# Pose-Group/FAMI-Pose

Hardware: AMD Instinct MI355X
Metric: train clips/sec (5-frame 384x288 HRNet-W48) (higher is better)
Workload: dtype f32

## Files before the change

### fami-pose_amd/csrc/conv.hip

```cpp
#include "common.h"
#include <type_traits>
#include <string.h>

#include "conv_epi.h"
extern "C" int fami_conv2d_fwd_bnin_ok(int N, int H, int W, int Ci, int Co);
#include "conv_pair.h"
int fami_pair_launch(const PairCapture& c, hipStream_t s);


struct ConvArgs {
  EpiBN e;
  int emode;
  const float* x;
  const float* wp;
  float* y;
  const float* bias;
  const float* addend;
  int N, Hi, Wi, Ci, Ho, Wo, Co;
  int kh, kw, sh, pad, dil;
  int KC, NTt, relu, accumulate, P;
  unsigned x_bytes, wp_bytes;
  int xcd;
  int prio;
  int par;
// ... 2387 lines not shown
        attr2 = true;                                                                                              \
      }                                                                                                            \
      hipLaunchKernelGGL((conv3x3_lds_kernel<T, nt, ksc, 1>), grid, dim3(256), lds, s, a);                         \
    } else                                                                                                         \
    hipLaunchKernelGGL((conv3x3_lds_kernel<T, nt, ksc>), grid, dim3(256), lds, s, a);                              \
    launched = true;                                                                                               \
  }
  FAMI_LDS_CASE(3, 1) FAMI_LDS_CASE(3, 2) FAMI_LDS_CASE(3, 3) FAMI_LDS_CASE(3, 4)
  FAMI_LDS_CASE(4, 1) FAMI_LDS_CASE(4, 2) FAMI_LDS_CASE(4, 3) FAMI_LDS_CASE(4, 4)
#undef FAMI_LDS_CASE
  if (!launched) return 0;
  hipError_t e = hipGetLastError();
  if (e != hipSuccess) {
    fami_set_error(name, hipGetErrorString(e));
    return FAMI_EHIP;
  }
  return 1;
}

static bool wgrad_lin_ok(int H, int W, int Ci, int Co, int kh, int kw, int stride, int pad, int dil) {
  return stride == 1 && 2 * pad == dil * (kh - 1) && 2 * pad == dil * (kw - 1) && kh * kw > 1 && kh * kw <= 9 && W >= 4 &&
         Ci % 16 == 0 && Co % 16 == 0;
}
static bool geom_ok(int kh, int kw, int stride, int pad, int dil) {
  return kh >= 1 && kw >= 1 && kh <= 7 && kw <= 7 && (stride == 1 || stride == 2) && pad >= 0 && dil >= 1;
}
static inline int out_dim(int i, int k, int stride, int pad, int dil) {
  return (i + 2 * pad - dil * (k - 1) - 1) / stride + 1;
}

extern "C" {
int fami_dcn_tune(int mode);
int fami_bn_tune_small(long elems);

int fami_conv_tune(int mt, int nt, int ks) {
  g_force_mt = mt; g_force_nt = nt; g_force_ks = ks;
  return FAMI_OK;
}
void fami_conv_stem_tune(int on);
int fami_conv_tune_lds(int on) {
  if (on == 9000 || on == 9001) {
    fami_conv_stem_tune(on - 9000);
    return FAMI_OK;
  }
  if (on < 0) fami_conv_stem_tune(-1);
  if (on == 10 || on == 11 || on == 20 || on == 21 || on == 30 || on == 31 || (on >= 40 && on <= 42) || (on >= 52 && on <= 54) || (on >= 60 && on <= 62) || on >= 100) {
    fami_conv_t4_tune(on);
    return FAMI_OK;
  }
  g_use_lds = on < 0 ? -1 : (on ? 1 : 0);
  g_lds_sim = on == 2;
  if (on < 0) fami_conv_t4_tune(-1);
  return FAMI_OK;
}
int fami_conv_tune_wgrad_lds(int on) {
  if (on >= 30000) {
    fami_wgrad_s3_tune(on - 30000);
    return FAMI_OK;
  }
  if (on >= 20000) {
    fami_wgrad16_tune(on - 20000);
    return FAMI_OK;
  }
  if (on >= 1000) {
    g_wgrad_ps = on - 1000;
    return FAMI_OK;
// ... 20 lines not shown
  if (on > 1) g_wgrad_nsub = on - 1;
  return FAMI_OK;
}
int fami_conv_tune_xcd(int mode) {
  g_xcd = mode < 0 ? -1 : (mode & 1);
  g_xcd_w = mode < 0 ? 1 : ((mode >> 1) & 1);
  return FAMI_OK;
}
int fami_conv_tune_stages(int stages) {
  if (stages == 120 || stages == 121) {
    g_prio = stages - 120;
    return FAMI_OK;
  }
  if (stages == 110 || stages == 111) {
    g_par = stages - 110;
    return FAMI_OK;
  }
  if (stages == 100 || stages == 101) {
    g_lin_conv = stages - 100;
    return FAMI_OK;
  }
  g_stages = (stages >= 2 && stages <= 4) ? stages : 0;
  return FAMI_OK;
}
int fami_tune_reset(void) {
  fami_conv_tune(0, 0, 0);
  fami_conv_tune_lds(-1);
  fami_conv_tune_wgrad_lds(-1);
  fami_conv_tune_xcd(-1);
  g_stages = 0; g_prio = 0; g_lin_conv = 1; g_par = 1;
  g_wgrad_ps = 0; g_wgrad_mt = 0;
  fami_dcn_tune(-1);
  fami_bn_tune_small(-1);
  return FAMI_OK;
}
int fami_tune_defaults(int f32_split) {
  if (f32_split >= 0) {
    fami_conv_t4_default_split(f32_split);
    fami_wgrad_s3_default(f32_split);
  }
  return fami_tune_reset();
}

long fami_packed_weight_elems(int Co, int Ci, int kh, int kw, int mode) {
  const int kd = mode == 0 ? Ci : Co, nd = mode == 0 ? Co : Ci;
  return pack16_elems(kd, nd, kh * kw) + pack32_elems(kd, nd, kh * kw) + fami_split_image_elems(kd, nd, kh * kw);
}

int fami_pack_conv_weight_f32(const float* w_oihw, float* wp, int Co, int Ci, int kh, int kw, int mode,
                              hipStream_t s) {
  FAMI_REQUIRE(w_oihw && wp && Co > 0 && Ci > 0 && (mode == 0 || mode == 1), "fami_pack_conv_weight_f32", "bad argument");
  const int kd = mode == 0 ? Ci : Co, nd = mode == 0 ? Co : Ci;
  const long total = pack16_elems(kd, nd, kh * kw) + pack32_elems(kd, nd, kh * kw);
  hipLaunchKernelGGL(pack_w_kernel, dim3(fami_ew_grid(total)), dim3(256), 0, s, w_oihw, wp, Co, Ci, kh * kw, mode);
  FAMI_CHECK_LAUNCH("fami_pack_conv_weight_f32");
  if (fami_split_image_elems(kd, nd, kh * kw) > 0) {
    fami_pack_split_single(w_oihw, wp + total, Co, Ci, kh * kw, mode, s);
    FAMI_CHECK_LAUNCH("fami_pack_conv_weight_f32/split");
  }
  return FAMI_OK;
}

static int conv_fwd_f32_impl(const char* nm, const float* x, const float* wp, const float* bias, const float* addend,
                             float* y, int N, int H, int W, int Ci, int Co, int kh, int kw, int stride, int pad, int dil,
                             int relu, int accumulate, const EpiBN& e, hipStream_t s, const XBN& xbn = xbn_none());
int fami_conv2d_fwd_f32(const float* x, const float* wp, const float* bias, const float* addend, float* y, int N,
// ... 35 lines not shown
                             int relu, int accumulate, const EpiBN& e, hipStream_t s, const XBN& xbn) {
  FAMI_REQUIRE(x && wp && y && N > 0 && H > 0 && W > 0 && Ci > 0 && Co > 0, nm, "bad argument");
  if (!geom_ok(kh, kw, stride, pad, dil)) {
    fami_set_error(nm, "unsupported geometry");
    return FAMI_ESHAPE;
  }
  ConvArgs a;
  a.e = e; a.emode = e.slots ? e.mode : 0;
  a.x = x; a.wp = wp; a.y = y; a.bias = bias; a.addend = addend;
  a.N = N; a.Hi = H; a.Wi = W; a.Ci = Ci;
  a.Ho = out_dim(H, kh, stride, pad, dil); a.Wo = out_dim(W, kw, stride, pad, dil); a.Co = Co;
  a.kh = kh; a.kw = kw; a.sh = stride == 2 ? 1 : 0; a.pad = pad; a.dil = dil;
  a.KC = fami_cdiv(Ci, 16); a.NTt = fami_cdiv(Co, 16); a.relu = relu; a.accumulate = accumulate;
  const long P = (long)N * a.Ho * a.Wo;
  const long xb = (long)N * H * W * Ci * 4, wb = (long)kh * kw * a.KC * a.NTt * 1024;
  FAMI_REQUIRE(P > 0 && P < (1L << 31) && xb < (1L << 31) && wb < (1L << 31), nm, "tensor >= 2 GiB");
  a.P = (int)P; a.x_bytes = (unsigned)xb; a.wp_bytes = (unsigned)wb;
  if (Ci == 3 && !addend && !xbn.on) {
    const int rc = fami_try_conv_stem1(2, x, wp, bias, y, N, H, W, Ci, Co, kh, kw, stride, pad, dil, a.NTt, relu, accumulate, 1, s, nm, e);
    if (rc != 0) return rc < 0 ? rc : FAMI_OK;
  }
  if (kh == 3 && kw == 3 && stride == 1 && pad == 1 && dil == 1 && !addend) {
    const int rc = try_conv3x3_lds<float>(x, wp, bias, y, N, H, W, Ci, Co, a.KC, a.NTt, +1, relu, accumulate, 1, s, nm, e, xbn);
    if (rc != 0) return rc < 0 ? rc : FAMI_OK;
  }
  if (kh == 3 && kw == 3 && stride == 1 && pad == dil && dil > 1 && !addend && !e.slots && !xbn.on && g_use_lds != 0) {
    const int rc = fami_try_conv3x3_t4_dil(2, x, wp, bias, y, N, H, W, Ci, Co, a.KC, a.NTt, +1, relu, accumulate, 1, dil, s, nm);
    if (rc != 0) return rc < 0 ? rc : FAMI_OK;
  }
  if (xbn.on) {
    fami_set_error(nm, "input BatchNorm needs the split-product 3x3 kernel (ask fami_conv2d_xbn_ok_f32 first)");
    return FAMI_ESHAPE;
  }
  return run_igemm(a, 0, s, nm);
}
extern "C" {

static int conv_dgrad_f32_impl(const char* nm, const float* dy, const float* wp, const float* addend, float* dx, int N,
                               int H, int W, int Ci, int Co, int kh, int kw, int stride, int pad, int dil, int accumulate,
                               const EpiBN& e, hipStream_t s);
int fami_conv2d_dgrad_f32(const float* dy, const float* wp, const float* addend, float* dx, int N, int H, int W,
                          int Ci, int Co, int kh, int kw, int stride, int pad, int dil, int accumulate,
                          hipStream_t s) {
  return conv_dgrad_f32_impl("fami_conv2d_dgrad_f32", dy, wp, addend, dx, N, H, W, Ci, Co, kh, kw, stride, pad, dil,
                             accumulate, epi_none(), s);
}
int fami_conv2d_dgrad_bnstats_f32(const float* dy, const float* wp, float* dx, int N, int H, int W, int Ci, int Co,
                                  int kh, int kw, int stride, int pad, int dil, int accumulate, const float* z,
                                  const float* yrelu, const float* mean, const float* invstd, const float* gamma,
                                  const float* beta, int relu, void* slots, hipStream_t s) {
  FAMI_REQUIRE(slots && z && mean && invstd && gamma && beta && (relu != 1 || yrelu) && relu >= 0 && relu <= 2,
               "fami_conv2d_dgrad_bnstats_f32", "bad argument");
  EpiBN e = epi_none();
  e.slots = reinterpret_cast<double*>(slots); e.ns = bn_slots(Ci); e.mode = 2; e.relu = relu; e.C = Ci;
  e.z = z; e.yr = yrelu; e.mean = mean; e.invstd = invstd; e.gamma = gamma; e.beta = beta;
  return conv_dgrad_f32_impl("fami_conv2d_dgrad_bnstats_f32", dy, wp, nullptr, dx, N, H, W, Ci, Co, kh, kw, stride, pad,
                             dil, accumulate, e, s);
}
}
static int conv_dgrad_f32_impl(const char* nm, const float* dy, const float* wp, const float* addend, float* dx, int N,
                               int H, int W, int Ci, int Co, int kh, int kw, int stride, int pad, int dil, int accumulate,
                               const EpiBN& e, hipStream_t s) {
  FAMI_REQUIRE(dy && wp && dx && N > 0 && H > 0 && W > 0 && Ci > 0 && Co > 0, nm, "bad argument");
  if (!geom_ok(kh, kw, stride, pad, dil)) {
    fami_set_error(nm, "unsupported geometry");
    return FAMI_ESHAPE;
  }
  ConvArgs a;
  a.e = e; a.emode = e.slots ? e.mode : 0;
  a.x = dy; a.wp = wp; a.y = dx; a.bias = nullptr; a.addend = addend;
  a.N = N; a.Hi = out_dim(H, kh, stride, pad, dil); a.Wi = out_dim(W, kw, stride, pad, dil); a.Ci = Co;
  a.Ho = H; a.Wo = W; a.Co = Ci;
  a.kh = kh; a.kw = kw; a.sh = stride == 2 ? 1 : 0; a.pad = pad; a.dil = dil;
  a.KC = fami_cdiv(Co, 16); a.NTt = fami_cdiv(Ci, 16); a.relu = 0; a.accumulate = accumulate;
  const long P = (long)N * H * W;
  const long xb = (long)N * a.Hi * a.Wi * Co * 4, wb = (long)kh * kw * a.KC * a.NTt * 1024;
  FAMI_REQUIRE(P > 0 && P < (1L << 31) && xb < (1L << 31) && wb < (1L << 31), nm, "tensor >= 2 GiB");
  a.P = (int)P; a.x_bytes = (unsigned)xb; a.wp_bytes = (unsigned)wb;
  if (kh == 3 && kw == 3 && stride == 1 && pad == 1 && dil == 1 && !addend) {
    const int rc = try_conv3x3_lds<float>(dy, wp, nullptr, dx, N, H, W, Co, Ci, a.KC, a.NTt, -1, 0, accumulate, 1, s, nm, e);
    if (rc != 0) return rc < 0 ? rc : FAMI_OK;
  }
  if (kh == 3 && kw == 3 && stride == 1 && pad == dil && dil > 1 && !addend && !e.slots && g_use_lds != 0) {
    const int rc = fami_try_conv3x3_t4_dil(2, dy, wp, nullptr, dx, N, H, W, Co, Ci, a.KC, a.NTt, -1, 0, accumulate, 1, dil, s, nm);
    if (rc != 0) return rc < 0 ? rc : FAMI_OK;
  }
  return run_igemm(a, 1, s, nm);
}
extern "C" {

struct WgradPlan { int MT, NT, ciBlocks, coBlocks, psplit, chunk, pertap, w8; long P; };
static bool wgrad_lin_ok(int H, int W, int Ci, int Co, int kh, int kw, int stride, int pad, int dil);
static WgradPlan wgrad_plan(int N, int H, int W, int Ci, int Co, int kh, int kw, int stride, int pad, int dil, int w8 = 0) {
  WgradPlan q;
  const int Ho = out_dim(H, kh, stride, pad, dil), Wo = out_dim(W, kw, stride, pad, dil);
  q.P = (long)N * Ho * Wo;
  q.MT = pick_small(fami_cdiv(Ci, 16));
  q.NT = pick_small(fami_cdiv(Co, 16));
  if (g_wgrad_mt > 0 && g_wgrad_mt <= q.MT) q.MT = g_wgrad_mt;
  q.ciBlocks = fami_cdiv(fami_cdiv(Ci, 16), q.MT);
  q.coBlocks = fami_cdiv(fami_cdiv(Co, 16), q.NT);
  q.pertap = (kh * kw > 1 && kh * kw <= 9) ? 1 : 0;
  const long by = q.pertap ? (long)q.ciBlocks * q.coBlocks : (long)kh * kw * q.ciBlocks * q.coBlocks;
  long ps = ((q.pertap ? (g_wgrad_ps ? g_wgrad_ps : 512) : 1024) + by - 1) / by;
  q.w8 = 0;
  if (w8 == 3) w8 = 256 / by >= 16 ? 2 : 1;
  if (w8 && q.pertap && kh * kw == 9 && ps >= 9) {
    q.w8 = w8;
    const long T = (g_wgrad_ps ? g_wgrad_ps : (w8 == 2 ? 256 : 512)) / by;
    ps = T * 8 / 9;
    while (ps > 1 && ps + (ps + 7) / 8 > T) --ps;
    if (ps < 1) ps = 1;
    if (w8 == 2) ps *= 2;
  }
  const long maxps = q.pertap ? (q.P + 63) / 64 : (q.P + 255) / 256;
  if (ps > maxps) ps = maxps;
  if (ps < 1) ps = 1;
// ... 62 lines not shown
  G = (P + chunk - 1) / chunk;
  q.G = (int)G;
  q.chunk = (int)chunk;
  q.xbytes = (int)((chunk + 2 * (W + 1)) * q.xrow);
  q.lds = ((size_t)q.xbytes + (size_t)chunk * q.yrow + 16) * 4;
  q.ok = P < (1L << 31) && G < 65536;
  return q;
}

int fami_conv2d_xbn_ok(int N, int H, int W, int Ci, int Co) {
  return (g_use_lds != 0 && g_wgrad_lds && fami_conv_t4_eligible16(N, H, W, Ci, Co) &&
          fami_wgrad16_slabs(N, H, W, Ci, Co, 3, 1, 1, 1) > 0) ? 1 : 0;
}
long fami_conv2d_wgrad_workspace(int N, int H, int W, int Ci, int Co, int kh, int kw, int stride, int pad, int dil) {
  if (!geom_ok(kh, kw, stride, pad, dil)) return -1;
  const WgradPlan q = wgrad_plan(N, H, W, Ci, Co, kh, kw, stride, pad, dil);
  long need = (long)q.psplit * Co * Ci * kh * kw * (long)sizeof(float);
  const WgradLdsPlan l = wgrad_lds_plan(N, H, W, Ci, Co, kh, kw, stride, pad, dil);
  if (l.ok) {
    const long nl = (long)l.G * Co * Ci * 9 * (long)sizeof(float);
    if (nl > need) need = nl;
  }
  const WgradLdsPlan f = wgrad_lds_plan_f32(N, H, W, Ci, Co, kh, kw, stride, pad, dil);
  if (f.ok) {
    const long nl = (long)f.G * Co * Ci * 9 * (long)sizeof(float);
    if (nl > need) need = nl;
  }
  if (kh == kw) {
    const long nl = fami_wgrad16_slabs(N, H, W, Ci, Co, kh, stride, pad, dil) * Co * Ci * kh * kw * (long)sizeof(float);
    if (nl > need) need = nl;
  }
  if (kh == 3 && kw == 3 && stride == 1 && pad == 1 && dil == 1) {
    const long nl = fami_wgrad_s3_slabs(N, H, W, Ci, Co) * Co * Ci * 9 * (long)sizeof(float);
    if (nl > need) need = nl;
  }
  return need;
}

}

template <typename T>
static int wgrad_impl(const T* x, const T* dy, float* dw, float* workspace, long ws_bytes, int N, int H, int W, int Ci,
                      int Co, int kh, int kw, int stride, int pad, int dil, int accumulate, hipStream_t s,
                      const char* nm) {
  FAMI_REQUIRE(x && dy && dw && workspace && N > 0 && H > 0 && W > 0 && Ci > 0 && Co > 0, nm, "bad argument");
  if (!geom_ok(kh, kw, stride, pad, dil)) {
    fami_set_error(nm, "unsupported geometry");
    return FAMI_ESHAPE;
  }
  const bool lin = std::is_same<T, float>::value && g_wgrad_lin && wgrad_lin_ok(H, W, Ci, Co, kh, kw, stride, pad, dil);
  const WgradPlan q = wgrad_plan(N, H, W, Ci, Co, kh, kw, stride, pad, dil, !lin ? 0 : (g_wgrad_lin == 1 ? 3 : (g_wgrad_lin == 3 ? 1 : (g_wgrad_lin == 4 ? 2 : 0))));
  const long need = (long)q.psplit * Co * Ci * kh * kw * (long)sizeof(float);
  FAMI_REQUIRE(ws_bytes >= need, nm, "workspace too small");
  FAMI_REQUIRE(q.P < (1L << 31), nm, "size out of range");
  WgradArgs<T> a;
  a.x = x; a.dy = dy; a.part = workspace;
  a.N = N; a.H = H; a.W = W; a.Ci = Ci;
  a.Ho = out_dim(H, kh, stride, pad, dil); a.Wo = out_dim(W, kw, stride, pad, dil); a.Co = Co;
  a.kh = kh; a.kw = kw; a.sh = stride == 2 ? 1 : 0; a.pad = pad; a.dil = dil;
  a.P = (int)q.P; a.chunk = q.chunk; a.ciBlocks = q.ciBlocks; a.coBlocks = q.coBlocks; a.xcd = g_xcd_w; a.prio = g_prio;
  const long xb = (long)N * H * W * Ci * (long)sizeof(T), yb = q.P * Co * (long)sizeof(T);
  FAMI_REQUIRE(xb < (1L << 31) && yb < (1L << 31), nm, "tensor >= 2 GiB");
  a.x_bytes = (unsigned)xb; a.dy_bytes = (unsigned)yb;
  if (q.pertap) {
    const dim3 grid(q.w8 ? q.psplit + (q.psplit + 7) / 8 : q.psplit, q.ciBlocks * q.coBlocks), block(q.w8 ? 512 * q.w8 : kh * kw * 64);
    const size_t lin_lds = q.w8 == 2 ? (size_t)8 * q.MT * q.NT * 1024 : 0;
// ... 104 lines not shown
  if (vec && g_force_mt) { MT = g_force_mt; NT = g_force_nt ? g_force_nt : NT; KS = g_force_ks ? g_force_ks : 1; }
  const int ST = g_stages ? g_stages : 2;
  int rc;
  if (mode == 0)
    rc = vec ? launch_igemm_h<H, 0, 1>(a, MT, NT, KS, ST, s) : launch_igemm_h<H, 0, 0>(a, MT, NT, KS, 2, s);
  else
    rc = vec ? launch_igemm_h<H, 1, 1>(a, MT, NT, KS, ST, s) : launch_igemm_h<H, 1, 0>(a, MT, NT, KS, 2, s);
  if (rc != 0) {
    fami_set_error(name, "no kernel instance for tile shape");
    return FAMI_ESHAPE;
  }
  FAMI_CHECK_LAUNCH(name);
  return FAMI_OK;
}

extern "C" {

static int wgrad_f32_entry(const float* x, const float* dy, float* dw, float* workspace, long ws_bytes, int N, int H,
                           int W, int Ci, int Co, int kh, int kw, int stride, int pad, int dil, int accumulate,
                           hipStream_t s, const XBN& xbn);
int fami_conv2d_wgrad_f32(const float* x, const float* dy, float* dw, float* workspace, long ws_bytes, int N, int H,
                          int W, int Ci, int Co, int kh, int kw, int stride, int pad, int dil, int accumulate,
                          hipStream_t s) {
  return wgrad_f32_entry(x, dy, dw, workspace, ws_bytes, N, H, W, Ci, Co, kh, kw, stride, pad, dil, accumulate, s, xbn_none());
}
static int wgrad_f32_entry(const float* x, const float* dy, float* dw, float* workspace, long ws_bytes, int N, int H,
                           int W, int Ci, int Co, int kh, int kw, int stride, int pad, int dil, int accumulate,
                           hipStream_t s, const XBN& xbn) {
  if (kh == 3 && kw == 3 && stride == 1 && pad == 1 && dil == 1 && x && dy && dw && workspace) {
    const int G = fami_try_wgrad_s3(x, dy, workspace, ws_bytes, N, H, W, Ci, Co, s, "fami_conv2d_wgrad_f32", xbn);
    if (G < 0) return G;
    if (G > 0) {
      launch_reduce_taps(workspace, dw, Co, Ci, 9, G, accumulate, s);
      FAMI_CHECK_LAUNCH("fami_conv2d_wgrad_f32/reduce");
      return FAMI_OK;
    }
  }
  if (xbn.on) {
    fami_set_error("fami_conv2d_wgrad_defer_xbn_f32", "input BatchNorm needs the split-product kernel (ask fami_conv2d_xbn_ok_f32 first)");
    return FAMI_ESHAPE;
  }
  WgradLdsPlan l = g_wgrad_lds_f32 ? wgrad_lds_plan_f32(N, H, W, Ci, Co, kh, kw, stride, pad, dil) : WgradLdsPlan{0};
  if (g_wgrad_lds_f32 == 2 && l.ok &&
      (l.ciBlocks * l.coBlocks < 64 || (g_wgrad_lin && wgrad_lin_ok(H, W, Ci, Co, kh, kw, stride, pad, dil))))
    l.ok = 0;
  if (l.ok && x && dy && dw && workspace && ((reinterpret_cast<uintptr_t>(x) | reinterpret_cast<uintptr_t>(dy)) & 15) == 0) {
    const long need = (long)l.G * Co * Ci * 9 * (long)sizeof(float);
    FAMI_REQUIRE(ws_bytes >= need, "fami_conv2d_wgrad_f32", "workspace too small");
    WgradLdsArgsF a;
    a.x = x; a.dy = dy; a.part = workspace;
    a.N = N; a.H = H; a.W = W; a.Ci = Ci; a.Co = Co; a.P = N * H * W;
    a.chunk = l.chunk; a.ciBlocks = l.ciBlocks; a.coBlocks = l.coBlocks; a.xcd = g_xcd_w;
    a.CiB = 16 * l.CIT; a.CoB = 16 * l.COT; a.xrow = l.xrow; a.yrow = l.yrow; a.xfloats = l.xbytes;
    const dim3 grid(l.G, l.ciBlocks * l.coBlocks);
    bool ok = false;
#define FAMI_WF_CASE(cit, cot)                                                                                        \
  if (l.CIT == cit && l.COT == cot) {                                                                                 \
    static bool attr = false;                                                                                         \
    if (!attr) {                                                                                                      \
      (void)hipFuncSetAttribute((const void*)conv_wgrad_lds_f32_kernel<cit, cot>, hipFuncAttributeMaxDynamicSharedMemorySize, 160 * 1024); \
      attr = true;                                                                                                    \
    }                                                                                                                 \
    hipLaunchKernelGGL((conv_wgrad_lds_f32_kernel<cit, cot>), grid, dim3(512), l.lds, s, a);                          \
    ok = true;                                                                                                        \
  }
    FAMI_WF_CASE(1, 1) FAMI_WF_CASE(1, 2) FAMI_WF_CASE(1, 3) FAMI_WF_CASE(1, 4) FAMI_WF_CASE(2, 1) FAMI_WF_CASE(2, 2)
// ... 444 lines not shown
```

### fami-pose_amd/csrc/conv_epi.h

```cpp
#pragma once
#include "common.h"

struct EpiBN {
  double* slots;
  int ns, mode, relu, C;
  const float* pivot_src;
  const void* z;
  const void* yr;
  const float *mean, *invstd, *gamma, *beta;
};
static inline EpiBN epi_none() {
  EpiBN e;
  e.slots = nullptr; e.ns = 1; e.mode = 0; e.relu = 0; e.C = 0; e.pivot_src = nullptr; e.z = nullptr; e.yr = nullptr;
  e.mean = e.invstd = e.gamma = e.beta = nullptr;
  return e;
}
#if defined(__HIP_DEVICE_COMPILE__)
typedef const __attribute__((address_space(4))) EpiBN* EpiPtr;
__device__ __forceinline__ EpiPtr epi_late(unsigned off) {
  const __attribute__((address_space(4))) char* k =
      (const __attribute__((address_space(4))) char*)__builtin_amdgcn_kernarg_segment_ptr() + off;
  asm volatile("" : "+s"(k) : : "memory");
  return (EpiPtr)k;
}
// ... 75 lines not shown
int fami_try_conv3x3_t4_dil(int half_kind, const void* x, const void* wp, const float* bias, void* y, int N, int H, int W, int Ci,
                            int Co, int KC, int NTt, int sgn, int relu, int accumulate, int out_f32, int dil, hipStream_t s,
                            const char* name);
void fami_conv_t4_tune(int on);
void fami_conv_t4_default_split(int on);
int fami_conv_t4_eligible16(int N, int H, int W, int Ci, int Co);
int fami_conv_t4_eligible_s3(int N, int H, int W, int Ci, int Co);

long fami_wgrad16_slabs(int N, int H, int W, int Ci, int Co, int k, int st, int pad, int dil);
int fami_try_wgrad16(int half_kind, const void* x, const void* dy, float* part, long ws_bytes, int N, int H, int W, int Ci,
                     int Co, int k, int st, int pad, int dil, hipStream_t s, const char* name, const XBN& xbn = xbn_none());
void fami_wgrad16_tune(int on);

long fami_wgrad_s3_slabs(int N, int H, int W, int Ci, int Co);
int fami_try_wgrad_s3(const float* x, const float* dy, float* part, long ws_bytes, int N, int H, int W, int Ci, int Co,
                      hipStream_t s, const char* name, const XBN& xbn = xbn_none());
void fami_wgrad_s3_tune(int on);
void fami_wgrad_s3_default(int on);

long fami_split_image_elems(int kd, int nd, int taps);
void fami_pack_split_single(const float* w_oihw, float* split, int Co, int Ci, int taps, int mode, hipStream_t s);
void fami_pack_split_batch(const float* params, float* packed, const void* desc, int n, hipStream_t s);
int fami_try_conv3x3_t5(int half_kind, const void* x, const void* wp, const float* bias, void* y, int N, int H, int W, int Ci,
                        int Co, int KC, int NTt, int sgn, int relu, int accumulate, int out_f32, hipStream_t s,
                        const char* name, const EpiBN& epi, const XBN& xbn);
void fami_conv_t5_tune(int on);
int fami_conv_t5_eligible_s3(int N, int H, int W, int Ci, int Co);

int fami_try_conv3x3_t6(int half_kind, const void* x, const void* wp, const float* bias, void* y, int N, int H, int W, int Ci,
                        int Co, int KC, int NTt, int sgn, int relu, int accumulate, int out_f32, hipStream_t s,
                        const char* name, const EpiBN& epi, const XBN& xbn);
extern "C" int fami_conv_t6_eligible(int N, int H, int W, int Ci, int Co);
void fami_conv_t6_tune(int on);
```

### fami-pose_amd/csrc/route.h

```cpp
#pragma once
#include "../../include/fami_route.h"
extern "C" fami_route_t* fami_rt(void);

#define g_dcn_gather (fami_rt()->dcn_gather)
#define g_dcn_abl (fami_rt()->dcn_abl)
#define g_dcn_win_r (fami_rt()->dcn_win_r)
#define g_dcn_ksplit (fami_rt()->dcn_ksplit)
#define g_dcn_pf (fami_rt()->dcn_pf)
#define g_dcn_bwd2 (fami_rt()->dcn_bwd2)
#define g_dcn_bwd2_cap (fami_rt()->dcn_bwd2_cap)
#define g_dcn_bwd2_stage (fami_rt()->dcn_bwd2_stage)
#define g_dcn_bwd_abl (fami_rt()->dcn_bwd_abl)
#define g_dcn_bwd_scatter (fami_rt()->dcn_bwd_scatter)
#define g_prio (fami_rt()->prio)
#define g_lin_conv (fami_rt()->lin_conv)
#define g_par (fami_rt()->par)
#define g_force_mt (fami_rt()->force_mt)
#define g_force_nt (fami_rt()->force_nt)
#define g_force_ks (fami_rt()->force_ks)
#define g_stages (fami_rt()->stages)
#define g_use32 (fami_rt()->use32)
#define g_xcd_w (fami_rt()->xcd_w)
#define g_xcd (fami_rt()->xcd)
#define g_use_lds (fami_rt()->use_lds)
// ... 28 lines not shown
#define g_t6_rows (fami_rt()->t6_rows)
#define g_t6_min_jobs (fami_rt()->t6_min_jobs)
#define g_t6_mt (fami_rt()->t6_mt)
#define g_t7_target (fami_rt()->t7_target)
#define g_use_t7 (fami_rt()->use_t7)
#define g_t7_rows (fami_rt()->t7_rows)
#define g_t7_c64 (fami_rt()->t7_c64)
#define g_bn_in (fami_rt()->bn_in)
#define g_bwd_pair (fami_rt()->bwd_pair)
#define g_pair_wg6_target (fami_rt()->pair_wg6_target)
#define g_wg6_s2 (fami_rt()->wg6_s2)
#define g_wg6_dil (fami_rt()->wg6_dil)
#define g_wg6_c42 (fami_rt()->wg6_c42)
#define g_wg6_c4 (fami_rt()->wg6_c4)
#define g_wg6 (fami_rt()->wg6)
#define g_wg6_nu (fami_rt()->wg6_nu)
#define g_wg6_target (fami_rt()->wg6_target)
#define g_wg6_target_c4 (fami_rt()->wg6_target_c4)
#define g_wg1 (fami_rt()->wg1)
#define g_wg1_target (fami_rt()->wg1_target)
#define g_wgs (fami_rt()->wgs)
#define g_wg16_abl (fami_rt()->wg16_abl)
#define g_wg16 (fami_rt()->wg16)
#define g_wg16_bt (fami_rt()->wg16_bt)
#define g_wg16_target (fami_rt()->wg16_target)
#define g_wg16_general (fami_rt()->wg16_general)
#define g_wg16_bt18 (fami_rt()->wg16_bt18)
#define g_wgs3 (fami_rt()->wgs3)
#define g_wgs3_bt (fami_rt()->wgs3_bt)
#define g_wgs3_target (fami_rt()->wgs3_target)
#define g_wgs3_default (fami_rt()->wgs3_default)
#define g_bn_small_elems (fami_rt()->bn_small_elems)
#define g_bn2_maxg (fami_rt()->bn2_maxg)

static inline void fami_route_set_defaults(fami_route_t* q) {
  q->size = (int)sizeof(fami_route_t);
  q->dcn_gather = -1;
  q->dcn_abl = 0;
  q->dcn_win_r = 0;
  q->dcn_ksplit = 1;
  q->dcn_pf = 0;
  q->dcn_bwd2 = 1;
  q->dcn_bwd2_cap = 36;
  q->dcn_bwd2_stage = 1;
  q->dcn_bwd_abl = 0;
  q->dcn_bwd_scatter = -1;
  q->prio = 0;
  q->lin_conv = 1;
  q->par = 1;
  q->force_mt = 0;
  q->force_nt = 0;
  q->force_ks = 0;
  q->stages = 0;
  q->use32 = 1;
  q->xcd_w = 1;
  q->xcd = -1;
  q->use_lds = -1;
  q->lds_sim = 0;
  q->wgrad_nsub = 2;
  q->wgrad_ps = 0;
  q->wgrad_mt = 0;
  q->wgrad_lds = 1;
  q->wgrad_lds_f32 = 2;
  q->wgrad_lin = 1;
  q->stem1 = 1;
  q->use_t4 = 1;
// ... 19 lines not shown
  q->t6_rows = 0;
  q->t6_min_jobs = 96;
  q->t6_mt = 0;
  q->t7_target = 240;
  q->use_t7 = 1;
  q->t7_rows = 0;
  q->t7_c64 = 1;
  q->bn_in = 1;
  q->bwd_pair = 1;
  q->pair_wg6_target = 64;
  q->wg6_s2 = 1;
  q->wg6_dil = 1;
  q->wg6_c42 = 1;
  q->wg6_c4 = 1;
  q->wg6 = 1;
  q->wg6_nu = 0;
  q->wg6_target = 80;
  q->wg6_target_c4 = 160;
  q->wg1 = 1;
  q->wg1_target = 192;
  q->wgs = 1;
  q->wg16_abl = 0;
  q->wg16 = 1;
  q->wg16_bt = 0;
  q->wg16_target = 0;
  q->wg16_general = 1;
  q->wg16_bt18 = 0;
  q->wgs3 = 1;
  q->wgs3_bt = 0;
  q->wgs3_target = 0;
  q->wgs3_default = 1;
  q->bn_small_elems = 32768;
  q->bn2_maxg = 512;
}
```

### include/fami.h

```cpp
#ifndef FAMI_H
#define FAMI_H
#ifdef __cplusplus
extern "C" {
#endif

typedef void* fami_stream_t;

#include "fami_route.h"
long fami_route_size(void);
int fami_route_init(fami_route_t* route);
int fami_route_bind(fami_route_t* route);

const char* fami_version(void);
const char* fami_last_error(void);
int fami_device_info(int device, int* info, char* name, int name_len);

int fami_conv_tune(int mt, int nt, int ks);
int fami_conv_tune_lds(int on);
int fami_conv_tune_wgrad_lds(int on);
int fami_conv_tune_xcd(int mode);
int fami_conv_tune_stages(int stages);
int fami_tune_reset(void);
int fami_tune_defaults(int f32_split);
int fami_conv_t5_eligible(int N, int H, int W, int Ci, int Co);
int fami_conv_t6_eligible(int N, int H, int W, int Ci, int Co);
long fami_packed_weight_elems(int Co, int Ci, int kh, int kw, int mode);
int fami_pack_conv_weight_f32(const float* w_oihw, float* wp, int Co, int Ci, int kh, int kw, int mode,
                              fami_stream_t stream);
int fami_pack_conv_weights_batch_f32(const float* params, float* packed, const void* desc, int n, fami_stream_t stream);
int fami_conv2d_fwd_f32(const float* x, const float* wp, const float* bias, const float* addend, float* y, int N,
                        int H, int W, int Ci, int Co, int kh, int kw, int stride, int pad, int dil, int relu,
                        int accumulate, fami_stream_t stream);
int fami_conv2d_dgrad_f32(const float* dy, const float* wp, const float* addend, float* dx, int N, int H, int W,
                          int Ci, int Co, int kh, int kw, int stride, int pad, int dil, int accumulate,
                          fami_stream_t stream);
int fami_conv2d_fwd_stats_f32(const float* x, const float* wp, const float* bias, float* y, int N, int H, int W, int Ci,
                              int Co, int kh, int kw, int stride, int pad, int dil, void* slots, const float* pivot_src,
                              fami_stream_t stream);
int fami_conv2d_dgrad_bnstats_f32(const float* dy, const float* wp, float* dx, int N, int H, int W, int Ci, int Co,
                                  int kh, int kw, int stride, int pad, int dil, int accumulate, const float* z,
                                  const float* yrelu, const float* mean, const float* invstd, const float* gamma,
                                  const float* beta, int relu, void* slots, fami_stream_t stream);
long fami_conv2d_wgrad_workspace(int N, int H, int W, int Ci, int Co, int kh, int kw, int stride, int pad, int dil);
int fami_wgrad_reduce_desc_longs(void);
int fami_wgrad_reduce_batch(const long* descs, int n, fami_stream_t stream);
int fami_conv2d_wgrad_defer_f32(const float* x, const float* dy, float* dw, float* workspace, long ws_bytes, int N,
                                int H, int W, int Ci, int Co, int kh, int kw, int stride, int pad, int dil,
                                int accumulate, long* desc_out, fami_stream_t stream);
int fami_conv2d_wgrad_f32(const float* x, const float* dy, float* dw, float* workspace, long ws_bytes, int N, int H,
                          int W, int Ci, int Co, int kh, int kw, int stride, int pad, int dil, int accumulate,
                          fami_stream_t stream);

long fami_bn_workspace(int C);
int fami_bn_stats_f32(const float* x, long P, int C, float* mean, float* invstd, float* running_mean,
                      float* running_var, float momentum, float eps, float* ws, fami_stream_t stream);
int fami_bn_train_fwd_f32(const float* x, const float* residual, float* y, const float* gamma, const float* beta,
                          float* mean, float* invstd, float* running_mean, float* running_var, long P, int C,
                          int relu, float momentum, float eps, float* ws, fami_stream_t stream);
// ... 446 lines not shown
```

### include/fami_route.h

```cpp
#ifndef FAMI_ROUTE_H
#define FAMI_ROUTE_H
#ifdef __cplusplus
extern "C" {
#endif

typedef struct fami_route_t {
  int size;
  int  dcn_gather;
  int  dcn_abl;
  int  dcn_win_r;
  int  dcn_ksplit;
  int  dcn_pf;
  int  dcn_bwd2;
  int  dcn_bwd2_cap;
  int  dcn_bwd2_stage;
  int  dcn_bwd_abl;
  int  dcn_bwd_scatter;
  int  prio;
  int  lin_conv;
  int  par;
  int  force_mt;
  int  force_nt;
  int  force_ks;
  int  stages;
// ... 32 lines not shown
  int  t6_rows;
  int  t6_min_jobs;
  int  t6_mt;
  int  t7_target;
  int  use_t7;
  int  t7_rows;
  int  t7_c64;
  int  bn_in;
  int  bwd_pair;
  int  pair_wg6_target;
  int  wg6_s2;
  int  wg6_dil;
  int  wg6_c42;
  int  wg6_c4;
  int  wg6;
  int  wg6_nu;
  int  wg6_target;
  int  wg6_target_c4;
  int  wg1;
  int  wg1_target;
  int  wgs;
  int  wg16_abl;
  int  wg16;
  int  wg16_bt;
  int  wg16_target;
  int  wg16_general;
  int  wg16_bt18;
  int  wgs3;
  int  wgs3_bt;
  int  wgs3_target;
  int  wgs3_default;
  long bn_small_elems;
  int  bn2_maxg;
} fami_route_t;

#ifdef __cplusplus
}
#endif
#endif
```

Baseline: 90.95.

## Add dedicated pointwise 1x1 conv kernels for forward, dgrad and weight gradient

Adds a specialized MFMA-based 1x1 convolution kernel with swizzled LDS staging and a fused bias/addend/relu/BN-stats epilogue, used for forward and data-gradient. It also adds a 1x1 weight-gradient kernel that writes per-block partial slabs, which are then reduced. By default only the weight-gradient path for large 64x64-channel layers is eligible; forward and dgrad need the tune mode raised. The aim is to replace the generic implicit-GEMM path for these layers at the cost of extra workspace and a reduction pass.

Measured after the change: 90.93. No clear change (-0.0%).

```diff
diff --git a/fami-pose_amd/csrc/conv.hip b/fami-pose_amd/csrc/conv.hip
--- a/fami-pose_amd/csrc/conv.hip
+++ b/fami-pose_amd/csrc/conv.hip
@@ -2443,6 +2443,7 @@
 extern "C" {
 int fami_dcn_tune(int mode);
 int fami_bn_tune_small(long elems);
+int fami_conv_pw_tune(int mode);
 
 int fami_conv_tune(int mt, int nt, int ks) {
   g_force_mt = mt; g_force_nt = nt; g_force_ks = ks;
@@ -2529,6 +2530,7 @@
   g_wgrad_ps = 0; g_wgrad_mt = 0;
   fami_dcn_tune(-1);
   fami_bn_tune_small(-1);
+  fami_conv_pw_tune(-1);
   return FAMI_OK;
 }
 int fami_tune_defaults(int f32_split) {
@@ -2630,6 +2632,10 @@
     fami_set_error(nm, "input BatchNorm needs the split-product 3x3 kernel (ask fami_conv2d_xbn_ok_f32 first)");
     return FAMI_ESHAPE;
   }
+  if (kh == 1 && kw == 1 && stride == 1 && pad == 0 && dil == 1 && pack32_elems(Ci, Co, 1) > 0) {
+    const int rc = fami_try_conv_pw(x, wp + pack16_elems(Ci, Co, 1), bias, addend, y, P, Ci, Co, relu, accumulate, 0, e, s, nm);
+    if (rc != 0) return rc < 0 ? rc : FAMI_OK;
+  }
   return run_igemm(a, 0, s, nm);
 }
 extern "C" {
@@ -2681,6 +2687,10 @@
   }
   if (kh == 3 && kw == 3 && stride == 1 && pad == dil && dil > 1 && !addend && !e.slots && g_use_lds != 0) {
     const int rc = fami_try_conv3x3_t4_dil(2, dy, wp, nullptr, dx, N, H, W, Co, Ci, a.KC, a.NTt, -1, 0, accumulate, 1, dil, s, nm);
+    if (rc != 0) return rc < 0 ? rc : FAMI_OK;
+  }
+  if (kh == 1 && kw == 1 && stride == 1 && pad == 0 && dil == 1 && pack32_elems(Co, Ci, 1) > 0 && !fami_pair_capture()) {
+    const int rc = fami_try_conv_pw(dy, wp + pack16_elems(Co, Ci, 1), nullptr, addend, dx, P, Co, Ci, 0, accumulate, 1, e, s, nm);
     if (rc != 0) return rc < 0 ? rc : FAMI_OK;
   }
   return run_igemm(a, 1, s, nm);
@@ -2809,6 +2819,10 @@
   }
   if (kh == 3 && kw == 3 && stride == 1 && pad == 1 && dil == 1) {
     const long nl = fami_wgrad_s3_slabs(N, H, W, Ci, Co) * Co * Ci * 9 * (long)sizeof(float);
+    if (nl > need) need = nl;
+  }
+  if (kh == 1 && kw == 1 && stride == 1 && pad == 0 && dil == 1) {
+    const long nl = fami_pw_wgrad_slabs((long)N * H * W, Ci, Co) * Co * Ci * (long)sizeof(float);
     if (nl > need) need = nl;
   }
   return need;
@@ -2979,6 +2993,15 @@
     if (G < 0) return G;
     if (G > 0) {
       launch_reduce_taps(workspace, dw, Co, Ci, 9, G, accumulate, s);
+      FAMI_CHECK_LAUNCH("fami_conv2d_wgrad_f32/reduce");
+      return FAMI_OK;
+    }
+  }
+  if (kh == 1 && kw == 1 && stride == 1 && pad == 0 && dil == 1 && x && dy && dw && workspace && !xbn.on && !fami_pair_capture()) {
+    const int G = fami_try_wgrad_pw(x, dy, workspace, ws_bytes, (long)N * H * W, Ci, Co, s, "fami_conv2d_wgrad_f32");
+    if (G < 0) return G;
+    if (G > 0) {
+      launch_reduce_plain(workspace, dw, Co, Ci, 1, G, accumulate, s);
       FAMI_CHECK_LAUNCH("fami_conv2d_wgrad_f32/reduce");
       return FAMI_OK;
     }
diff --git a/fami-pose_amd/csrc/conv_epi.h b/fami-pose_amd/csrc/conv_epi.h
--- a/fami-pose_amd/csrc/conv_epi.h
+++ b/fami-pose_amd/csrc/conv_epi.h
@@ -131,3 +131,9 @@
                         const char* name, const EpiBN& epi, const XBN& xbn);
 extern "C" int fami_conv_t6_eligible(int N, int H, int W, int Ci, int Co);
 void fami_conv_t6_tune(int on);
+
+int fami_try_conv_pw(const float* x, const float* wp32, const float* bias, const float* addend, float* y, long P, int K,
+                     int N, int relu, int accumulate, int dir, const EpiBN& epi, hipStream_t s, const char* name);
+long fami_pw_wgrad_slabs(long P, int Ci, int Co);
+int fami_try_wgrad_pw(const float* x, const float* dy, float* part, long ws_bytes, long P, int Ci, int Co, hipStream_t s,
+                      const char* name);
diff --git a/fami-pose_amd/csrc/conv_pw.hip b/fami-pose_amd/csrc/conv_pw.hip
--- /dev/null
+++ b/fami-pose_amd/csrc/conv_pw.hip
@@ -0,0 +1,373 @@
+#include "common.h"
+#include "conv_epi.h"
+
+typedef float f32x16 __attribute__((ext_vector_type(16)));
+#define PW_OOB 0x80000000u
+
+
+#define PW_MP 128
+struct PwArgs {
+  EpiBN e;
+  int emode;
+  const float* x;
+  const float* wp;
+  float* y;
+  const float* bias;
+  const float* addend;
+  int P, K, N, KC8, NT32, relu, accumulate;
+  unsigned x_bytes, wp_bytes;
+};
+
+template <int KFIX>
+__global__ __launch_bounds__(256, 2) void conv_pw_f32(PwArgs p) {
+  __shared__ __attribute__((aligned(16))) float lds[PW_MP * 64 + 64 * 64 + 512];
+  float* xs = lds;
+  float* ws = lds + PW_MP * 64;
+  float* ered = ws + 64 * 64;
+  const int t = threadIdx.x;
+  const int lane = t & 63;
+  const int wave = __builtin_amdgcn_readfirstlane(t >> 6);
+  const int col = lane & 31, h = lane >> 5;
+  const int K = KFIX ? KFIX : p.K;
+  const int nkc = (K + 63) >> 6, nnc = (p.NT32 + 1) >> 1;
+  const int m0 = blockIdx.x * PW_MP;
+  const int emode = p.emode;
+  const __amdgpu_buffer_rsrc_t rx = __builtin_amdgcn_make_buffer_rsrc((void*)p.x, 0, (int)p.x_bytes, 0x00020000);
+  const __amdgpu_buffer_rsrc_t rw = __builtin_amdgcn_make_buffer_rsrc((void*)p.wp, 0, (int)p.wp_bytes, 0x00020000);
+
+  u32x4 xr[8], wr[4];
+  const int spx = t >> 4, sc4 = t & 15;
+  const unsigned xv = (unsigned)(((m0 + spx) * K + sc4 * 4) * 4);
+  auto load_x = [&](int kc) {
+    const bool cv = kc * 64 + sc4 * 4 < K;
+#pragma unroll
+    for (int i = 0; i < 8; ++i) {
+      const unsigned o = cv ? xv + (unsigned)((i * 16 * K + kc * 64) * 4) : PW_OOB;
+      xr[i] = __builtin_amdgcn_raw_buffer_load_b128(rx, o, 0, 0);
+    }
+  };
+  auto store_x = [&]() {
+#pragma unroll
+    for (int i = 0; i < 8; ++i) {
+      const int px = i * 16 + spx;
+      *reinterpret_cast<u32x4*>(xs + px * 64 + ((sc4 ^ (px & 15)) << 2)) = xr[i];
+    }
+  };
+  auto load_w = [&](int nc, int kc) {
+#pragma unroll
+    for (int i = 0; i < 4; ++i) {
+      const int idx = i * 256 + t;
+      const int k8 = kc * 8 + (idx >> 7), ntg = nc * 2 + ((idx >> 6) & 1);
+      const unsigned o = (k8 < p.KC8 && ntg < p.NT32) ? (unsigned)(((k8 * p.NT32 + ntg) * 64 + (idx & 63)) * 16) : PW_OOB;
+      wr[i] = __builtin_amdgcn_raw_buffer_load_b128(rw, o, 0, 0);
+    }
+  };
+  auto store_w = [&]() {
+#pragma unroll
+    for (int i = 0; i < 4; ++i) *reinterpret_cast<u32x4*>(ws + (i * 256 + t) * 4) = wr[i];
+  };
+
+  f32x16 acc[2], tot[2];
+  const float* xfrag = xs + (wave * 32 + col) * 64;
+  const int xsw = col & 15;
+
+  const bool restage_x = nkc > 1;
+  load_x(0);
+  load_w(0, 0);
+  const int nsteps = nnc * nkc;
+  int nc = 0, kc = 0;
+#pragma unroll 1
+  for (int step = 0; step < nsteps; ++step) {
+    __syncthreads();
+    if (restage_x || step == 0) store_x();
+    store_w();
+    __syncthreads();
+    int nc1 = nc, kc1 = kc + 1;
+    if (kc1 == nkc) { kc1 = 0; ++nc1; }
+    if (step + 1 < nsteps) {
+      if (restage_x) load_x(kc1);
+      load_w(nc1, kc1);
+    }
+#pragma unroll
+    for (int r = 0; r < 16; ++r) acc[0][r] = acc[1][r] = 0.f;
+#pragma unroll
+    for (int ks = 0; ks < 8; ++ks) {
+      const f32x4 a = *reinterpret_cast<const f32x4*>(xfrag + (((ks * 2 + h) ^ xsw) << 2));
+      const f32x4 b0 = *reinterpret_cast<const f32x4*>(ws + ((ks * 2 + 0) * 64 + lane) * 4);
+      const f32x4 b1 = *reinterpret_cast<const f32x4*>(ws + ((ks * 2 + 1) * 64 + lane) * 4);
+#pragma unroll
+      for (int u = 0; u < 4; ++u) {
+        acc[0] = __builtin_amdgcn_mfma_f32_32x32x2f32(b0[u], a[u], acc[0], 0, 0, 0);
+        acc[1] = __builtin_amdgcn_mfma_f32_32x32x2f32(b1[u], a[u], acc[1], 0, 0, 0);
+      }
+    }
+    if (restage_x) {
+      if (kc == 0) {
+        tot[0] = acc[0];
+        tot[1] = acc[1];
+      } else {
+        tot[0] += acc[0];
+        tot[1] += acc[1];
+      }
+      if (kc == nkc - 1) {
+        acc[0] = tot[0];
+        acc[1] = tot[1];
+      }
+    }
+    if (kc == nkc - 1) {
+#pragma unroll
+      for (int nt = 0; nt < 2; ++nt) {
+        if (nc * 2 + nt >= p.NT32) break;
+        __syncthreads();
+        {
+          const int lp = wave * 32 + col;
+#pragma unroll
+          for (int q = 0; q < 4; ++q) {
+            const f32x4 v = {acc[nt][4 * q], acc[nt][4 * q + 1], acc[nt][4 * q + 2], acc[nt][4 * q + 3]};
+            *reinterpret_cast<f32x4*>(ws + lp * 32 + (((2 * q + h) ^ (lp & 7)) << 2)) = v;
+          }
+        }
+        __syncthreads();
+        const int u = t & 7;
+        const int co = (nc * 2 + nt) * 32 + u * 4;
+        f32x4 bv = {0.f, 0.f, 0.f, 0.f}, ek = {0.f, 0.f, 0.f, 0.f}, es = {0.f, 0.f, 0.f, 0.f}, eq = {0.f, 0.f, 0.f, 0.f};
+        if (p.bias) {
+#pragma unroll
+          for (int r = 0; r < 4; ++r) bv[r] = p.bias[co + r];
+        }
+        if (emode) {
+          EpiPtr e = epi_late(__builtin_offsetof(PwArgs, e));
+          const float* ps = e->pivot_src;
+          if (ps) {
+#pragma unroll
+            for (int r = 0; r < 4; ++r) ek[r] = ps[co + r];
+          }
+        }
+#pragma unroll
+        for (int pass = 0; pass < 4; ++pass) {
+          const int lp = pass * 32 + (t >> 3);
+          const int m = m0 + lp;
+          if (m >= p.P) continue;
+          f32x4 v = *reinterpret_cast<const f32x4*>(ws + lp * 32 + ((u ^ (lp & 7)) << 2));
+          const long idx = (long)m * p.N + co;
+          v += bv;
+          if (p.addend) v += *reinterpret_cast<const f32x4*>(p.addend + idx);
+          if (p.relu) {
+#pragma unroll
+            for (int r = 0; r < 4; ++r) v[r] = fmaxf(v[r], 0.f);
+          }
+          if (p.accumulate) v += *reinterpret_cast<const f32x4*>(p.y + idx);
+          if (emode) {
+            const f32x4 d = v - ek;
+            es += d;
+#pragma unroll
+            for (int r = 0; r < 4; ++r) eq[r] = __builtin_fmaf(d[r], d[r], eq[r]);
+          }
+          *reinterpret_cast<f32x4*>(p.y + idx) = v;
+        }
+        if (emode) {
+#pragma unroll
+          for (int r = 0; r < 4; ++r) {
+#pragma unroll
+            for (int o = 8; o < 64; o <<= 1) {
+              es[r] += __shfl_xor(es[r], o, 64);
+              eq[r] += __shfl_xor(eq[r], o, 64);
+            }
+          }
+          if (lane < 8) {
+            *reinterpret_cast<f32x4*>(ered + wave * 128 + nt * 32 + u * 4) = es;
+            *reinterpret_cast<f32x4*>(ered + wave * 128 + 64 + nt * 32 + u * 4) = eq;
+          }
+        }
+      }
+      if (emode) {
+        __syncthreads();
+        if (t < 128) {
+          EpiPtr e = epi_late(__builtin_offsetof(PwArgs, e));
+          const int st = t >> 6, c = t & 63;
+          const int co = nc * 64 + c;
+          if (co < p.N) {
+            const int eC = e->C;
+            double* srow = e->slots + (long)((int)blockIdx.x % e->ns) * 2 * eC;
+            const float v = (ered[t] + ered[128 + t]) + (ered[256 + t] + ered[384 + t]);
+            unsafeAtomicAdd(srow + st * eC + co, (double)v);
+            if (st == 0 && blockIdx.x == 0) bn_slots_pivot(e->slots, eC)[co] = e->pivot_src ? e->pivot_src[co] : 0.f;
+          }
+        }
+      }
+    }
+    nc = nc1;
+    kc = kc1;
+  }
+}
+
+static bool pw_shape_ok(long P, int Ci, int Co, int dir) {
+  if (P <= 0 || Ci <= 0 || Co <= 0) return false;
+  if (dir == 2) {
+    return Ci % 32 == 0 && Co % 32 == 0 && (Ci / 32) * (Co / 32) <= 16 && Ci + Co <= 512 && (P + 128) * (Ci > Co ? Ci : Co) * 4 < (1L << 31);
+  }
+  const int K = dir == 0 ? Ci : Co, N = dir == 0 ? Co : Ci;
+  return K % 16 == 0 && N % 32 == 0 && N >= 64 && (P + PW_MP) * (K > N ? K : N) * 4 < (1L << 31);
+}
+static bool pw_eligible(long P, int Ci, int Co, int dir) {
+  if (g_pw_f32 == 0 || !pw_shape_ok(P, Ci, Co, dir)) return false;
+  if (g_pw_f32 >= 2) return true;
+  return dir == 2 && P >= 65536 && Ci == 64 && Co == 64;
+}
+
+extern "C" {
+int fami_conv_pw_tune(int mode) {
+  g_pw_f32 = mode < 0 ? 1 : (mode > 2 ? 2 : mode);
+  return FAMI_OK;
+}
+int fami_conv_pw_eligible_f32(int N, int H, int W, int Ci, int Co, int direction) {
+  if (direction < 0 || direction > 2 || N <= 0 || H <= 0 || W <= 0) return 0;
+  return pw_eligible((long)N * H * W, Ci, Co, direction) ? 1 : 0;
+}
+}
+
+int fami_try_conv_pw(const float* x, const float* wp32, const float* bias, const float* addend, float* y, long P, int K,
+                     int N, int relu, int accumulate, int dir, const EpiBN& epi, hipStream_t s, const char* name) {
+  if (!pw_eligible(P, dir == 0 ? K : N, dir == 0 ? N : K, dir)) return 0;
+  if (epi.slots && epi.mode != 1) return 0;
+  const uintptr_t al = reinterpret_cast<uintptr_t>(x) | reinterpret_cast<uintptr_t>(y) | reinterpret_cast<uintptr_t>(wp32) |
+                       reinterpret_cast<uintptr_t>(addend);
+  if (al & 15) return 0;
+  PwArgs a;
+  a.e = epi; a.emode = epi.slots ? 1 : 0;
+  a.x = x; a.wp = wp32; a.y = y; a.bias = bias; a.addend = addend;
+  a.P = (int)P; a.K = K; a.N = N; a.KC8 = K / 8; a.NT32 = N / 32; a.relu = relu; a.accumulate = accumulate;
+  a.x_bytes = (unsigned)(P * K * 4); a.wp_bytes = (unsigned)((long)a.KC8 * a.NT32 * 1024);
+  const dim3 grid(fami_cdiv(P, PW_MP));
+  if (K == 64) hipLaunchKernelGGL(conv_pw_f32<64>, grid, dim3(256), 0, s, a);
+  else if (K == 256) hipLaunchKernelGGL(conv_pw_f32<256>, grid, dim3(256), 0, s, a);
+  else hipLaunchKernelGGL(conv_pw_f32<0>, grid, dim3(256), 0, s, a);
+  FAMI_CHECK_LAUNCH(name);
+  return 1;
+}
+
+struct PwWgArgs {
+  const float* x;
+  const float* dy;
+  float* part;
+  int P, Ci, Co, run, cpx;
+  unsigned x_bytes, dy_bytes;
+};
+#define PW_WG_NLD 16
+
+template <int TPW>
+__global__ __launch_bounds__(256) void conv_pw_wgrad_f32(PwWgArgs p) {
+  extern __shared__ __attribute__((aligned(16))) float wlds[];
+  const int t = threadIdx.x;
+  const int lane = t & 63;
+  const int wave = __builtin_amdgcn_readfirstlane(t >> 6);
+  const int col = lane & 31, h = lane >> 5;
+  const int Ci = p.Ci, Co = p.Co, cpx = p.cpx;
+  const int q0 = blockIdx.x * p.run;
+  const int qend = min(q0 + p.run, p.P);
+  float* xt = wlds;
+  float* yt = wlds + cpx * Ci;
+  const __amdgpu_buffer_rsrc_t rx = __builtin_amdgcn_make_buffer_rsrc((void*)p.x, 0, (int)p.x_bytes, 0x00020000);
+  const __amdgpu_buffer_rsrc_t ry = __builtin_amdgcn_make_buffer_rsrc((void*)p.dy, 0, (int)p.dy_bytes, 0x00020000);
+  const int nx = (cpx * Ci) >> 10, nld = nx + ((cpx * Co) >> 10);
+  const unsigned tv = (unsigned)t * 16u;
+
+  u32x4 sr[PW_WG_NLD];
+  auto load = [&](int q) {
+    const unsigned xq = (unsigned)(q * Ci * 4), yq = (unsigned)(q * Co * 4);
+#pragma unroll
+    for (int i = 0; i < PW_WG_NLD; ++i) {
+      if (i < nld) {
+        if (i < nx) sr[i] = __builtin_amdgcn_raw_buffer_load_b128(rx, tv + (xq + (unsigned)i * 4096u), 0, 0);
+        else sr[i] = __builtin_amdgcn_raw_buffer_load_b128(ry, tv + (yq + (unsigned)(i - nx) * 4096u), 0, 0);
+      }
+    }
+  };
+  auto store = [&]() {
+#pragma unroll
+    for (int i = 0; i < PW_WG_NLD; ++i) {
+      if (i < nld) *reinterpret_cast<u32x4*>(wlds + (i * 256 + t) * 4) = sr[i];
+    }
+  };
+
+  const int TN = Ci >> 5, T = TN * (Co >> 5);
+  int aoff[TPW], boff[TPW];
+  f32x16 acc[TPW];
+#pragma unroll
+  for (int j = 0; j < TPW; ++j) {
+    const int tid = min(wave + 4 * j, T - 1);
+    const int tm = tid / TN, tn = tid - tm * TN;
+    aoff[j] = h * Co + tm * 32 + col;
+    boff[j] = h * Ci + tn * 32 + col;
+#pragma unroll
+    for (int r = 0; r < 16; ++r) acc[j][r] = 0.f;
+  }
+
+  load(q0);
+#pragma unroll 1
+  for (int q = q0; q < qend; q += cpx) {
+    __syncthreads();
+    store();
+    __syncthreads();
+    if (q + cpx < qend) load(q + cpx);
+#pragma unroll 1
+    for (int sb = 0; sb < cpx; sb += 32) {
+      const float* yb = yt + sb * Co;
+      const float* xb = xt + sb * Ci;
+#pragma unroll
+      for (int s2 = 0; s2 < 32; s2 += 2) {
+#pragma unroll
+        for (int j = 0; j < TPW; ++j) {
+          const float a = yb[s2 * Co + aoff[j]];
+          const float b = xb[s2 * Ci + boff[j]];
+          acc[j] = __builtin_amdgcn_mfma_f32_32x32x2f32(a, b, acc[j], 0, 0, 0);
+        }
+      }
+    }
+  }
+  float* slab = p.part + (long)blockIdx.x * Co * Ci;
+#pragma unroll
+  for (int j = 0; j < TPW; ++j) {
+    const int tid = wave + 4 * j;
+    if (tid >= T) break;
+    const int tm = tid / TN, tn = tid - tm * TN;
+#pragma unroll
+    for (int r = 0; r < 16; ++r) {
+      const int co = tm * 32 + (r & 3) + 8 * (r >> 2) + 4 * h;
+      slab[(long)co * Ci + tn * 32 + col] = acc[j][r];
+    }
+  }
+}
+
+struct PwWgPlan { int G, run, cpx, tpw; };
+static PwWgPlan pw_wgrad_plan(long P, int Ci, int Co) {
+  PwWgPlan q;
+  int f = 512 / (Ci + Co);
+  f = f >= 4 ? 4 : (f >= 2 ? 2 : 1);
+  q.cpx = 32 * f;
+  const long per = (P + 255) / 256;
+  q.run = (int)((per + q.cpx - 1) / q.cpx * q.cpx);
+  q.G = (int)((P + q.run - 1) / q.run);
+  const int T = (Ci / 32) * (Co / 32);
+  q.tpw = T <= 4 ? 1 : (T <= 8 ? 2 : 4);
+  return q;
+}
+long fami_pw_wgrad_slabs(long P, int Ci, int Co) {
+  return pw_eligible(P, Ci, Co, 2) ? pw_wgrad_plan(P, Ci, Co).G : 0;
+}
+int fami_try_wgrad_pw(const float* x, const float* dy, float* part, long ws_bytes, long P, int Ci, int Co, hipStream_t s,
+                      const char* name) {
+  if (!pw_eligible(P, Ci, Co, 2)) return 0;
+  if ((reinterpret_cast<uintptr_t>(x) | reinterpret_cast<uintptr_t>(dy) | reinterpret_cast<uintptr_t>(part)) & 15) return 0;
+  const PwWgPlan q = pw_wgrad_plan(P, Ci, Co);
+  FAMI_REQUIRE(ws_bytes >= (long)q.G * Co * Ci * 4, name, "workspace too small");
+  PwWgArgs a;
+  a.x = x; a.dy = dy; a.part = part; a.P = (int)P; a.Ci = Ci; a.Co = Co; a.run = q.run; a.cpx = q.cpx;
+  a.x_bytes = (unsigned)(P * Ci * 4); a.dy_bytes = (unsigned)(P * Co * 4);
+  const size_t lds = (size_t)q.cpx * (Ci + Co) * 4;
+  if (q.tpw == 1) hipLaunchKernelGGL(conv_pw_wgrad_f32<1>, dim3(q.G), dim3(256), lds, s, a);
+  else if (q.tpw == 2) hipLaunchKernelGGL(conv_pw_wgrad_f32<2>, dim3(q.G), dim3(256), lds, s, a);
+  else hipLaunchKernelGGL(conv_pw_wgrad_f32<4>, dim3(q.G), dim3(256), lds, s, a);
+  FAMI_CHECK_LAUNCH(name);
+  return q.G;
+}
diff --git a/fami-pose_amd/csrc/route.h b/fami-pose_amd/csrc/route.h
--- a/fami-pose_amd/csrc/route.h
+++ b/fami-pose_amd/csrc/route.h
@@ -84,6 +84,7 @@
 #define g_wgs3_default (fami_rt()->wgs3_default)
 #define g_bn_small_elems (fami_rt()->bn_small_elems)
 #define g_bn2_maxg (fami_rt()->bn2_maxg)
+#define g_pw_f32 (fami_rt()->pw_f32)
 
 static inline void fami_route_set_defaults(fami_route_t* q) {
   q->size = (int)sizeof(fami_route_t);
@@ -169,4 +170,5 @@
   q->wgs3_default = 1;
   q->bn_small_elems = 32768;
   q->bn2_maxg = 512;
+  q->pw_f32 = 1;
 }
diff --git a/include/fami.h b/include/fami.h
--- a/include/fami.h
+++ b/include/fami.h
@@ -24,6 +24,8 @@
 int fami_tune_defaults(int f32_split);
 int fami_conv_t5_eligible(int N, int H, int W, int Ci, int Co);
 int fami_conv_t6_eligible(int N, int H, int W, int Ci, int Co);
+int fami_conv_pw_tune(int mode);
+int fami_conv_pw_eligible_f32(int N, int H, int W, int Ci, int Co, int direction);
 long fami_packed_weight_elems(int Co, int Ci, int kh, int kw, int mode);
 int fami_pack_conv_weight_f32(const float* w_oihw, float* wp, int Co, int Ci, int kh, int kw, int mode,
                               fami_stream_t stream);
diff --git a/include/fami_route.h b/include/fami_route.h
--- a/include/fami_route.h
+++ b/include/fami_route.h
@@ -88,6 +88,7 @@
   int  wgs3_default;
   long bn_small_elems;
   int  bn2_maxg;
+  int  pw_f32;
 } fami_route_t;
 
 #ifdef __cplusplus
```
